# foundation-model-stack/fms-fsdp

Measured on AMD Instinct MI355X. Metric: tokens/sec (aggregate), higher is better.
Workload: dtype bf16; 1 GPU; model=llama2_7b, global_batch=2, seq_len=4096, parallelism=hsdp1

## Files before the change

fms_fsdp_amd/models/llama.py:

```python

import math
import os
from dataclasses import dataclass


import torch
import torch.nn as nn

from fms_fsdp_amd import ops


@dataclass
class LlamaConfig:
    src_vocab_size: int = 32000
    emb_dim: int = 4096
    nheads: int = 32
    kvheads: int = 0
    nlayers: int = 32
    hidden_grow_factor: float = 8 / 3
    multiple_of: int = 256
    max_expected_seq_len: int = 4096
    rope_theta: float = 10000.0
    norm_eps: float = 1e-6

# ... 47 lines not shown
        return freqs.cos(), freqs.sin()

    def get(self, seqlen, device):
        if seqlen > self.cos.shape[0]:
            cos, sin = self._build(seqlen)
            self.cos, self.sin = cos.to(device), sin.to(device)
        return self.cos[:seqlen], self.sin[:seqlen]

    def reset_parameters(self):
        cos, sin = self._build(self.max_seq_len)
        with torch.no_grad():
            self.cos.copy_(cos)
            self.sin.copy_(sin)


class Attention(nn.Module):
    def __init__(self, cfg: LlamaConfig):
        super().__init__()
        self.nheads = cfg.nheads
        self.kvheads = cfg.kvheads
        self.head_dim = cfg.head_dim
        qkv_out = (cfg.nheads + 2 * cfg.kvheads) * cfg.head_dim
        self.qkv = nn.Linear(cfg.emb_dim, qkv_out, bias=False)
        self.proj = nn.Linear(cfg.emb_dim, cfg.emb_dim, bias=False)
        self.qkv.weight._direct_wgrad = True
        self.proj.weight._direct_wgrad = True

    def _project_out(self, o2, residual, b, s):
        if getattr(self, "_disable_fused_residual", False):
            out = self.proj(o2.reshape(b * s, -1)).view(b, s, -1)
            return out if residual is None else out + residual
        return ops.linear_flat(o2.view(b, s, -1), self.proj.weight, residual)

    def forward(self, x, cos, sin, cache=None, residual=None, doc_mask=None):
        b, s, _ = x.shape
        if getattr(self, "_disable_fused_residual", False):
            qkv = self.qkv(x)
        else:
            qkv = ops.linear_flat(x, self.qkv.weight)
        if (cache is None and qkv.is_cuda and s % 128 == 0
                and self.head_dim in (64, 128)
                and qkv.dtype == torch.bfloat16
                and os.environ.get("FMS_AMD_ALLOW_TORCH_SDPA") != "1"
                and os.environ.get("FMS_AMD_DISABLE_FUSED_QKV") != "1"):
            o = ops.qkv_rope_attention(qkv, cos, sin, self.nheads,
                                       self.kvheads, self.head_dim,
                                       doc_mask=doc_mask)
            return self._project_out(o.reshape(b, s, -1), residual, b, s)
        q, k, v = qkv.split(
            [self.nheads * self.head_dim,
             self.kvheads * self.head_dim,
             self.kvheads * self.head_dim], dim=-1)
        q = q.view(b, s, self.nheads, self.head_dim)
        k = k.view(b, s, self.kvheads, self.head_dim)
        v = v.view(b, s, self.kvheads, self.head_dim)
        q, k = ops.rope_apply(q, k, cos, sin)
        if cache is not None:
            import torch.nn.functional as F
            if cache.get("k") is not None:
                k = torch.cat([cache["k"], k], dim=1)
                v = torch.cat([cache["v"], v], dim=1)
            cache["k"], cache["v"] = k, v
            o = F.scaled_dot_product_attention(
                q.transpose(1, 2), k.transpose(1, 2), v.transpose(1, 2),
                is_causal=(s == k.shape[1]),
                enable_gqa=(self.kvheads != self.nheads)).transpose(1, 2)
        else:
            o = ops.attention_causal(q, k, v, doc_mask=doc_mask)
        return self._project_out(o.reshape(b, s, -1), residual, b, s)

    def reset_parameters(self):
        for lin in (self.qkv, self.proj):
            nn.init.trunc_normal_(lin.weight, mean=0.0, std=0.02)


class SwiGLU(nn.Module):
    def __init__(self, cfg: LlamaConfig):
        super().__init__()
        self.hidden_dim = cfg.hidden_dim
        self.wg1 = nn.Linear(cfg.emb_dim, 2 * cfg.hidden_dim, bias=False)
        self.w2 = nn.Linear(cfg.hidden_dim, cfg.emb_dim, bias=False)
        self.wg1.weight._direct_wgrad = True
        self.w2.weight._direct_wgrad = True

    def forward(self, x, residual=None):
        if getattr(self, "_disable_fused_residual", False):
            gu = self.wg1(x)
            h = ops.swiglu(gu)
            out = self.w2(h)
            return out if residual is None else out + residual.view_as(out)
        gu = ops.linear_flat(x, self.wg1.weight)
        h = ops.swiglu(gu)
        return ops.linear_flat(h, self.w2.weight, residual)

    def reset_parameters(self):
        for lin in (self.wg1, self.w2):
            nn.init.trunc_normal_(lin.weight, mean=0.0, std=0.02)


class LlamaBlock(nn.Module):

    def __init__(self, cfg: LlamaConfig):
        super().__init__()
        self.attn_norm = RMSNorm(cfg.emb_dim, cfg.norm_eps)
        self.attn = Attention(cfg)
        self.mlp_norm = RMSNorm(cfg.emb_dim, cfg.norm_eps)
        self.mlp = SwiGLU(cfg)
        self.attn_norm.weight._direct_wgrad = True
        self.mlp_norm.weight._direct_wgrad = True

    def forward(self, x, cos, sin, cache=None, doc_mask=None):
        if cache is None and getattr(self, "_ac_enabled", False) \
                and torch.is_grad_enabled():
            return torch.utils.checkpoint.checkpoint(
                self._forward_impl, x, cos, sin, None, doc_mask,
                use_reentrant=False)
        return self._forward_impl(x, cos, sin, cache, doc_mask)

    def _forward_impl(self, x, cos, sin, cache=None, doc_mask=None):
        n, x_res = ops.rmsnorm_residual(x, self.attn_norm.weight,
                                        self.attn_norm.eps)
        h = self.attn(n, cos, sin, cache, residual=x_res, doc_mask=doc_mask)
        n, h_res = ops.rmsnorm_residual(h, self.mlp_norm.weight,
                                        self.mlp_norm.eps)
        return self.mlp(n, residual=h_res)

    def reset_parameters(self):
        for m in (self.attn_norm, self.attn, self.mlp_norm, self.mlp):
            m.reset_parameters()


class Llama(nn.Module):
    def __init__(self, cfg: LlamaConfig):
        super().__init__()
        self.config = cfg
        self.embedding = nn.Embedding(cfg.src_vocab_size, cfg.emb_dim)
        self.rot_emb = RotaryEmbedding(cfg.head_dim, cfg.max_expected_seq_len, cfg.rope_theta)
        self.layers = nn.ModuleList([LlamaBlock(cfg) for _ in range(cfg.nlayers)])
        self.norm = RMSNorm(cfg.emb_dim, cfg.norm_eps)
        self.norm.weight._direct_wgrad = True
        self.lm_head = nn.Linear(cfg.emb_dim, cfg.src_vocab_size, bias=False)
        self.doc_mask_token = None

    def forward(self, tokens, labels=None, include_embeds=False,
                doc_mask=None):
        b, s = tokens.shape
        if doc_mask is None and self.doc_mask_token is not None:
            doc_mask = ops.doc_mask_from_tokens(tokens, self.doc_mask_token)
        x = self.embedding(tokens)
        cos, sin = self.rot_emb.get(s, x.device)
        for layer in self.layers:
            x = layer(x, cos, sin, doc_mask=doc_mask)
        x = self.norm(x)
        if labels is not None:
            loss = ops.linear_cross_entropy(x, self.lm_head.weight, labels)
            return (loss, x) if include_embeds else loss
        logits = self.lm_head(x)
        return (logits, x) if include_embeds else logits

    @torch.no_grad()
    def generate(self, input_ids, max_new_tokens, temperature=1.0,
                 do_sample=True, include_embeds=False):
        b, s0 = input_ids.shape
        caches = [{} for _ in self.layers]
        tokens = input_ids
        embeds = []
# ... 38 lines not shown
```

fms_fsdp_amd/ops/__init__.py:

```python

import os
from typing import NamedTuple

import torch

from . import reference


_C = None
_C_err = None
try:
    from fms_fsdp_amd import _C
except ImportError as e:
    _C_err = e


def _require_ext(op):
    if _C is None:
        raise RuntimeError(
            f"fms_fsdp_amd._C HIP extension is required for {op} on GPU but "
            f"could not be imported ({_C_err}). Build it with "
            f"`python setup.py build_ext --inplace` (PYTORCH_ROCM_ARCH=gfx950)."
        )
    return _C
# ... 114 lines not shown
        weight = _WgradSinkFn.apply(weight)
    return reference.rmsnorm(x, weight, eps)


def rmsnorm_residual(x, weight, eps=1e-6):
    out = _rmsnorm_dispatch(_RMSNormResidualFn, x, weight, eps)
    if out is not None:
        return out
    if _direct_wgrad_on(weight):
        weight = _WgradSinkFn.apply(weight)
    return reference.rmsnorm(x, weight, eps), x


class _AddRMSNormFn(torch.autograd.Function):

    @staticmethod
    def forward(ctx, x, res, weight, eps):
        ext = _require_ext("add_rmsnorm")
        x2d = x.contiguous().view(-1, x.shape[-1])
        r2d = res.contiguous().view_as(x2d)
        y, s, rinv = ext.add_rmsnorm_fwd(x2d, r2d, weight, eps)
        ctx.save_for_backward(s, weight, rinv)
        ctx.shape = x.shape
        return y.view(x.shape), s.view(x.shape)

    @staticmethod
    def backward(ctx, dy, ds):
        s, weight, rinv = ctx.saved_tensors
        dx, dw = _C.rmsnorm_bwd(dy.contiguous().view_as(s), s, weight, rinv,
                                ds.contiguous().view_as(s))
        dx = dx.view(ctx.shape)
        return dx, dx, dw.to(weight.dtype), None


def add_rmsnorm(x, res, weight, eps=1e-6):
    if x.is_cuda and x.dtype != torch.float32:
        if x.dtype == torch.float16:
            y, s = _AddRMSNormFn.apply(x.bfloat16(), res.bfloat16(),
                                       weight.bfloat16(), eps)
            return y.half(), s.half()
        return _AddRMSNormFn.apply(x, res, weight, eps)
    s = (x.float() + res.float()).to(x.dtype)
    return reference.rmsnorm(s, weight, eps), s


def _row_view_ok(t):
    return (t.dim() == 4 and t.stride(3) == 1 and t.stride(2) == t.shape[3]
            and t.stride(1) >= t.shape[2] * t.shape[3]
            and t.stride(0) == t.shape[1] * t.stride(1))


def _as_row_view(t):
    return t if _row_view_ok(t) else t.contiguous()


class _RoPEFn(torch.autograd.Function):
    @staticmethod
    def forward(ctx, q, k, cos, sin):
        ext = _require_ext("rope")
        cos = cos.float().contiguous()
        sin = sin.float().contiguous()
        qo, ko = ext.rope_fwd(_as_row_view(q), _as_row_view(k), cos, sin,
                              False)
        ctx.save_for_backward(cos, sin)
        return qo, ko

    @staticmethod
    def backward(ctx, dq, dk):
        cos, sin = ctx.saved_tensors
        dqo, dko = _C.rope_fwd(_as_row_view(dq), _as_row_view(dk), cos, sin,
                               True)
        return dqo, dko, None, None


def rope_apply(q, k, cos, sin):
    if q.is_cuda and q.dtype != torch.float32:
        if q.dtype == torch.float16:
            qo, ko = _RoPEFn.apply(q.bfloat16(), k.bfloat16(), cos, sin)
            return qo.half(), ko.half()
        return _RoPEFn.apply(q, k, cos, sin)
    return reference.rope_apply(q, k, cos, sin)


class _DirectWgradLinearFn(torch.autograd.Function):
    @staticmethod
    def forward(ctx, x, weight, residual):
        ctx.save_for_backward(x, weight)
        ctx.gview = weight._flat_grad_view
        ctx.wobj = weight
        ctx.cb = getattr(weight, "_wgrad_done", None)
        ctx.res_shape = residual.shape if residual is not None else None
        x2 = x.reshape(-1, x.shape[-1])
        if residual is not None:
            y = torch.addmm(residual.reshape(x2.shape[0], -1), x2,
                            weight.t())
        else:
            y = x2 @ weight.t()
        return y.view(*x.shape[:-1], weight.shape[0])

    @staticmethod
    def backward(ctx, dy):
        x, w = ctx.saved_tensors
        dy2 = dy.reshape(-1, dy.shape[-1])
        x2 = x.reshape(-1, x.shape[-1])
        dx = (dy2 @ w).view(x.shape)
        if getattr(ctx.wobj, "_wgrad_fresh", False):
            torch.addmm(ctx.gview, dy2.t(), x2, beta=0, out=ctx.gview)
            ctx.wobj._wgrad_fresh = False
        else:
            ctx.gview.addmm_(dy2.t(), x2)
        if ctx.cb is not None:
            ctx.cb()
        dres = dy.reshape(ctx.res_shape) if ctx.res_shape is not None else None
        return dx, None, dres


def linear_flat(x, weight, residual=None):
    if (getattr(weight, "_flat_grad_view", None) is not None
            and weight.requires_grad and torch.is_grad_enabled()):
        return _DirectWgradLinearFn.apply(x, weight, residual)
    x2 = x.reshape(-1, x.shape[-1])
    if residual is not None:
        y = torch.addmm(residual.reshape(x2.shape[0], -1), x2, weight.t())
    else:
        y = x2 @ weight.t()
    return y.view(*x.shape[:-1], weight.shape[0])


class DocMask(NamedTuple):
    start: torch.Tensor
    end: torch.Tensor


def doc_mask_from_starts(doc_start):
    b, s = doc_start.shape
    start = doc_start.long()
    pos = torch.arange(s, device=start.device).expand(b, s)
    opens = torch.where(start == pos, pos, torch.full_like(pos, s))
    nxt = torch.cat([opens[:, 1:], torch.full_like(pos[:, :1], s)], dim=1)
    end = torch.cummin(nxt.flip(1), dim=1).values.flip(1)
    return DocMask(start.int().contiguous(), end.int().contiguous())


def doc_mask_from_tokens(tokens, eos_token):
    b, s = tokens.shape
    pos = torch.arange(s, device=tokens.device).expand(b, s)
    after = torch.where(tokens == eos_token, pos + 1, torch.zeros_like(pos))
    prev = torch.cat([torch.zeros_like(after[:, :1]), after[:, :-1]], dim=1)
    return doc_mask_from_starts(torch.cummax(prev, dim=1).values)


def _pad_doc_mask(doc_mask, s_pad):
    b, s = doc_mask.start.shape
    if s == s_pad:
        return doc_mask.start.contiguous(), doc_mask.end.contiguous()
    start = doc_mask.start.new_full((b, s_pad), s)
    end = doc_mask.end.new_full((b, s_pad), s_pad)
    start[:, :s] = doc_mask.start
    end[:, :s] = doc_mask.end
    return start, end


class _FlashAttnFn(torch.autograd.Function):

    @staticmethod
    def _pad(t, s_pad):
        b, s, h, d = t.shape
        if s == s_pad:
            return t.contiguous()
        out = torch.zeros(b, s_pad, h, d, dtype=t.dtype, device=t.device)
        out[:, :s] = t
        return out

    @staticmethod
    def forward(ctx, q, k, v, doc_start=None, doc_end=None):
        ext = _require_ext("attention")
        s = q.shape[1]
        s_pad = (s + 127) // 128 * 128
        qp = _FlashAttnFn._pad(q, s_pad)
        kp = _FlashAttnFn._pad(k, s_pad)
        vp = _FlashAttnFn._pad(v, s_pad)
        if doc_start is None:
            o, lse = ext.attn_fwd(qp, kp, vp)
            ctx.save_for_backward(qp, kp, vp, o, lse)
        else:
            o, lse = ext.attn_fwd_doc(qp, kp, vp, doc_start)
            ctx.save_for_backward(qp, kp, vp, o, lse, doc_start, doc_end)
        ctx.s = s
# ... 353 lines not shown
```

fms_fsdp_amd/ops/hip/bindings.cpp:

```cpp
#include <torch/extension.h>
#include <c10/hip/HIPStream.h>
#include <hip/hip_runtime_api.h>

#include <string>
#include <tuple>
#include <vector>

#include "attn_ws.h"

using torch::Tensor;

extern "C" {
void launch_rmsnorm_fwd(const void*, const void*, void*, float*, int, int,
                        float, hipStream_t);
void launch_rmsnorm_bwd(const void*, const void*, const void*, const float*,
                        const void*, void*, float*, int, int, hipStream_t);
void launch_add_rmsnorm_fwd(const void*, const void*, const void*, void*,
                            void*, float*, int, int, float, hipStream_t);
int rmsnorm_bwd_grid(int);
int rmsnorm_bwd_nparts(int, int);
void launch_rmsnorm_bwd_fused(const void*, const void*, const void*,
                              const float*, const void*, void*, float*, int,
                              float*, void*, int, int, int, hipStream_t);
void launch_rmsnorm_dw_store(const float*, void*, int, int, hipStream_t);
void launch_rope(const void*, void*, const float*, const float*, int, int,
                 int, int, int, long long, long long, hipStream_t);
void launch_swiglu_fwd(const void*, void*, long long, int, hipStream_t);
void launch_swiglu_bwd(const void*, const void*, void*, long long, int,
                       hipStream_t);
void launch_ce_fwd_bwd(void*, const long long*, float*, const float*,
                       long long, int, int, hipStream_t);
void launch_adamw(float*, const void*, int, float*, float*, void*, int,
                  long long, float, float, float, float, float, float, float,
                  const float*, hipStream_t);
void launch_sqnorm(const void*, int, float*, long long, hipStream_t);
void launch_attn_fwd(const void*, const void*, const void*, void*, float*,
                     int, int, int, int, int, float, long long, hipStream_t);
void launch_attn_bwd(const void*, const void*, const void*, const void*,
                     const void*, const float*, void*, void*, void*, float*,
                     void*, int, int, int, int, int, float, int,
                     long long, long long, hipStream_t);
void launch_attn_fwd_doc(const void*, const void*, const void*, void*, float*,
                         const int*, int, int, int, int, int, float,
                         long long, hipStream_t);
void launch_attn_bwd_doc(const void*, const void*, const void*, const void*,
                         const void*, const float*, void*, void*, void*,
                         float*, const int*, const int*, int, int, int, int,
                         int, float, int, long long, long long, hipStream_t);
void launch_attn_bwd_delta(const void*, const void*, float*, int, int, int,
                           int, hipStream_t);
int attn_sched_mode(int);
int attn_dkv_mode(int);
long long attn_bwd_ws_limit(long long);
void launch_cconv_fwd(const void*, const void*, const float*, void*, int,
                      int, int, int, hipStream_t);
void launch_cconv_bwd(const void*, const void*, const void*, const float*,
                      void*, void*, float*, float*, int, int, int, int,
                      hipStream_t);
int launch_gemm_nt(const void*, const void*, void*, int, int, int,
                   hipStream_t);
void launch_segsum_exp_fwd(const float*, void*, long long, int, hipStream_t);
void launch_segsum_exp_bwd(const void*, const float*, float*, long long, int,
                           hipStream_t);
void launch_ssd_prep_fwd(const void*, const float*, const float*, float*,
                         float*, long long, int, int, long long, hipStream_t);
void launch_ssd_prep_bwd(const float*, const float*, const void*,
                         const float*, const float*, void*, float*, float*,
                         long long, int, int, long long, long long,
                         hipStream_t);
void launch_ssd_xdt_fwd(const void*, const float*, const float*, void*, void*,
                        long long, int, int, int, long long, hipStream_t);
void launch_ssd_xdt_bwd(const void*, const void*, const void*, const float*,
                        const float*, void*, float*, float*, long long, int,
                        int, int, long long, long long, hipStream_t);
void launch_ssd_sl_fwd(const float*, const void*, void*, long long, int, int,
                       int, hipStream_t);
void launch_ssd_sl_bwd(const void*, const void*, const float*, void*, float*,
                       long long, int, int, int, hipStream_t);
void launch_ssd_ygate_fwd(const void*, const void*, const float*, const void*,
                          const float*, const void*, void*, long long, int,
                          int, int, int, long long, long long, hipStream_t);
void launch_ssd_ygate_bwd(const void*, const void*, const void*, const float*,
                          const void*, const float*, const void*, void*,
                          void*, float*, void*, float*, void*, long long, int,
                          int, int, int, long long, long long, long long,
                          long long, hipStream_t);
}

static hipStream_t cur_stream() {
  return c10::hip::getCurrentHIPStream().stream();
}

#define CHECK_BF16_CONTIG(t)                                        \
  TORCH_CHECK(t.scalar_type() == torch::kBFloat16, #t " must be bf16"); \
  TORCH_CHECK(t.is_contiguous(), #t " must be contiguous");

std::tuple<Tensor, Tensor> rmsnorm_fwd(Tensor x, Tensor w, double eps) {
  CHECK_BF16_CONTIG(x);
  CHECK_BF16_CONTIG(w);
  const int rows = x.size(0), H = x.size(1);
  TORCH_CHECK(H % 8 == 0, "H must be divisible by 8");
  auto y = torch::empty_like(x);
  auto rinv = torch::empty({rows}, x.options().dtype(torch::kFloat32));
  launch_rmsnorm_fwd(x.data_ptr(), w.data_ptr(), y.data_ptr(),
                     rinv.data_ptr<float>(), rows, H, (float)eps,
                     cur_stream());
  return {y, rinv};
}

static void check_rmsnorm_bwd_args(const Tensor& dy, const Tensor& x,
                                   const Tensor& w, const Tensor& rinv,
                                   const c10::optional<Tensor>& dextra) {
  CHECK_BF16_CONTIG(dy);
  CHECK_BF16_CONTIG(x);
  CHECK_BF16_CONTIG(w);
  TORCH_CHECK(x.dim() == 2 && dy.sizes() == x.sizes(),
              "dy and x must be (rows, H)");
  const int rows = x.size(0), H = x.size(1);
  TORCH_CHECK(H % 8 == 0, "H must be divisible by 8");
  TORCH_CHECK(w.numel() == H, "w must have H elements");
  TORCH_CHECK(rinv.scalar_type() == torch::kFloat32 && rinv.is_contiguous() &&
                  rinv.numel() == rows,
              "rinv must be fp32 with one element per row");
  if (dextra.has_value()) {
    TORCH_CHECK(dextra->scalar_type() == torch::kBFloat16 &&
                    dextra->is_contiguous() && dextra->sizes() == x.sizes(),
                "dextra must have x's shape and dtype");
  }
}

std::tuple<Tensor, Tensor> rmsnorm_bwd(Tensor dy, Tensor x, Tensor w,
                                       Tensor rinv,
                                       c10::optional<Tensor> dextra) {
  check_rmsnorm_bwd_args(dy, x, w, rinv, dextra);
  const int rows = x.size(0), H = x.size(1);
  const void* de = dextra.has_value() ? dextra->data_ptr() : nullptr;
  auto f32 = x.options().dtype(torch::kFloat32);
  auto dx = torch::empty_like(x);
  const int nparts = rmsnorm_bwd_nparts(rows, H);
  if (nparts == 0) {
    auto dw = torch::zeros({H}, f32);
    launch_rmsnorm_bwd(dy.data_ptr(), x.data_ptr(), w.data_ptr(),
                       rinv.data_ptr<float>(), de, dx.data_ptr(),
// ... 341 lines not shown
  } else {
    dv = out_bf16 ? torch::empty({b, s, kvh, d}, opts)
                  : torch::zeros({b, s, kvh, d}, opts);
  }
  auto delta = torch::empty({b, h, s}, q.options().dtype(torch::kFloat32));
  const float scale = 1.f / sqrtf((float)d);
  launch_attn_bwd_doc(do_.data_ptr(), q.data_ptr(), k.data_ptr(),
                      v.data_ptr(), o.data_ptr(), lse.data_ptr<float>(),
                      dq.data_ptr(), dk.data_ptr(), dv.data_ptr(),
                      delta.data_ptr<float>(), doc_start.data_ptr<int>(),
                      doc_end.data_ptr<int>(), b, s, h, kvh, d, scale,
                      out_bf16 ? 1 : 0, vs, dvs, cur_stream());
  if (out_bf16) return {dq, dk, dv};
  return {dq, dk.to(torch::kBFloat16), dv.to(torch::kBFloat16)};
}

Tensor cconv_fwd(Tensor x, Tensor w, Tensor bias) {
  CHECK_BF16_CONTIG(x);
  CHECK_BF16_CONTIG(w);
  const int b = x.size(0), l = x.size(1), c = x.size(2);
  const int W = w.size(1);
  TORCH_CHECK(c % 8 == 0 && W >= 2 && W <= 4);
  TORCH_CHECK(bias.scalar_type() == torch::kFloat32);
  auto y = torch::empty_like(x);
  launch_cconv_fwd(x.data_ptr(), w.data_ptr(), bias.data_ptr<float>(),
                   y.data_ptr(), b * l, l, c, W, cur_stream());
  return y;
}

std::tuple<Tensor, Tensor, Tensor> cconv_bwd(Tensor dy, Tensor x, Tensor w,
                                             Tensor bias) {
  CHECK_BF16_CONTIG(dy);
  CHECK_BF16_CONTIG(x);
  const int b = x.size(0), l = x.size(1), c = x.size(2);
  const int W = w.size(1);
  TORCH_CHECK(c % 8 == 0 && W >= 2 && W <= 4);
  auto g = torch::empty_like(x);
  auto dx = torch::empty_like(x);
  auto dw = torch::zeros({c, W}, x.options().dtype(torch::kFloat32));
  auto db = torch::zeros({c}, x.options().dtype(torch::kFloat32));
  launch_cconv_bwd(dy.data_ptr(), x.data_ptr(), w.data_ptr(),
                   bias.data_ptr<float>(), g.data_ptr(), dx.data_ptr(),
                   dw.data_ptr<float>(), db.data_ptr<float>(), b * l, l, c, W,
                   cur_stream());
  return {dx, dw, db};
}

Tensor segsum_exp_fwd(Tensor cs) {
  TORCH_CHECK(cs.scalar_type() == torch::kFloat32 && cs.is_contiguous());
  const long long N = cs.numel() / cs.size(-1);
  const int Q = cs.size(-1);
  TORCH_CHECK(Q % 8 == 0);
  std::vector<int64_t> shape(cs.sizes().begin(), cs.sizes().end());
  shape.push_back(Q);
  auto out = torch::empty(shape, cs.options().dtype(torch::kBFloat16));
  launch_segsum_exp_fwd(cs.data_ptr<float>(), out.data_ptr(), N, Q,
                        cur_stream());
  return out;
}

Tensor segsum_exp_bwd(Tensor g, Tensor cs) {
  CHECK_BF16_CONTIG(g);
  const long long N = cs.numel() / cs.size(-1);
  const int Q = cs.size(-1);
  auto dcs = torch::empty_like(cs);
  launch_segsum_exp_bwd(g.data_ptr(), cs.data_ptr<float>(),
                        dcs.data_ptr<float>(), N, Q, cur_stream());
  return dcs;
}


Tensor gemm_nt(Tensor A, Tensor B) {
  CHECK_BF16_CONTIG(A);
  CHECK_BF16_CONTIG(B);
  const int M = A.size(0), K = A.size(1), N = B.size(1);
  TORCH_CHECK(B.size(0) == K);
  auto C = torch::empty({M, N}, A.options());
  const int rc = launch_gemm_nt(A.data_ptr(), B.data_ptr(), C.data_ptr(), M,
                                N, K, cur_stream());
  TORCH_CHECK(rc == 0, "gemm_nt: shape not supported (M%256/N%256/K%64)");
  return C;
}

static long long slice_stride(const Tensor& t, const char* nm) {
  TORCH_CHECK(t.scalar_type() == torch::kBFloat16, nm, " must be bf16");
  TORCH_CHECK(t.dim() == 2 && t.stride(1) == 1, nm, " must be 2-D row-major");
  return t.stride(0);
}

static void check_nq(const Tensor& t, long long N, long long Q,
                     const char* nm) {
  TORCH_CHECK(t.scalar_type() == torch::kFloat32, nm, " must be fp32");
  TORCH_CHECK(t.is_contiguous(), nm, " must be contiguous");
  TORCH_CHECK(t.dim() == 2 && t.size(0) == N && t.size(1) == Q, nm,
              " must have shape (rows/Q*H, Q)");
}

static void check_bf16_numel(const Tensor& t, long long numel,
                             const char* nm) {
  TORCH_CHECK(t.scalar_type() == torch::kBFloat16, nm, " must be bf16");
  TORCH_CHECK(t.is_contiguous(), nm, " must be contiguous");
  TORCH_CHECK(t.numel() == numel, nm, " has the wrong element count");
}

static void check_head_vec(const Tensor& t, long long H, const char* nm) {
  TORCH_CHECK(t.scalar_type() == torch::kFloat32 && t.is_contiguous() &&
                  t.numel() == H,
              nm, " must be contiguous fp32 with H elements");
}

static long long check_xslice(const Tensor& t, int64_t H, int64_t P,
                              int64_t Q, const char* nm) {
  const long long st = slice_stride(t, nm);
  TORCH_CHECK(H > 0 && P > 0 && P % 8 == 0, "P must be divisible by 8");
  TORCH_CHECK(Q > 0 && Q % 8 == 0, "Q must be divisible by 8");
  TORCH_CHECK(t.size(1) == H * P, nm, " must have H*P columns");
  TORCH_CHECK(t.size(0) % Q == 0, nm, " rows must be a multiple of Q");
  return st;
}

static void check_prep_q(long long rows, int64_t Q) {
  TORCH_CHECK(Q > 0 && Q <= 256 && Q % 64 == 0 && rows % Q == 0,
              "Q must be 64, 128, 192 or 256 and divide the row count");
}

std::tuple<Tensor, Tensor> ssd_prep_fwd(Tensor dt, Tensor bias, Tensor alog,
                                        int64_t Q) {
  const long long sdt = slice_stride(dt, "dt");
  const long long rows = dt.size(0);
  const int H = dt.size(1);
  check_prep_q(rows, Q);
  check_head_vec(bias, H, "bias");
  check_head_vec(alog, H, "alog");
  const long long N = rows / Q * H;
  auto opt = dt.options().dtype(torch::kFloat32);
  auto dtf = torch::empty({N, Q}, opt);
  auto dacs = torch::empty({N, Q}, opt);
  launch_ssd_prep_fwd(dt.data_ptr(), bias.data_ptr<float>(),
                      alog.data_ptr<float>(), dtf.data_ptr<float>(),
                      dacs.data_ptr<float>(), N, H, (int)Q, sdt,
                      cur_stream());
  return {dtf, dacs};
}

std::tuple<Tensor, Tensor, Tensor> ssd_prep_bwd(Tensor ddtf, Tensor ddacs,
                                                Tensor dt, Tensor bias,
                                                Tensor alog, int64_t Q) {
  const long long sdt = slice_stride(dt, "dt");
  const long long rows = dt.size(0);
  const int H = dt.size(1);
  check_prep_q(rows, Q);
  check_head_vec(bias, H, "bias");
  check_head_vec(alog, H, "alog");
  const long long N = rows / Q * H;
  check_nq(ddtf, N, Q, "ddtf");
  check_nq(ddacs, N, Q, "ddacs");
  auto ddt = torch::empty({rows, (long long)H},
                          dt.options().dtype(torch::kBFloat16));
  auto dbias = torch::zeros({H}, dt.options().dtype(torch::kFloat32));
  auto dalog = torch::zeros({H}, dt.options().dtype(torch::kFloat32));
  launch_ssd_prep_bwd(ddtf.data_ptr<float>(), ddacs.data_ptr<float>(),
                      dt.data_ptr(), bias.data_ptr<float>(),
                      alog.data_ptr<float>(), ddt.data_ptr(),
                      dbias.data_ptr<float>(), dalog.data_ptr<float>(), N, H,
                      (int)Q, sdt, H, cur_stream());
  return {ddt, dbias, dalog};
// ... 69 lines not shown
  const int Q = check_sl(dacs, scores, H, G);
  const long long N = dacs.size(0);
  check_bf16_numel(g, N * Q * Q, "g");
  auto dsh = torch::empty({N, (long long)Q, (long long)Q}, g.options());
  auto dcs = torch::zeros_like(dacs);
  launch_ssd_sl_bwd(g.data_ptr(), scores.data_ptr(), dacs.data_ptr<float>(),
                    dsh.data_ptr(), dcs.data_ptr<float>(), N, (int)H, (int)G,
                    Q, cur_stream());
  return {dsh, dcs};
}

static void check_ygate(const Tensor& ydiag, const Tensor& yoff,
                        const Tensor& dacs, const Tensor& x, const Tensor& Dp,
                        const Tensor& z, int64_t H, int64_t G, int64_t Q) {
  TORCH_CHECK(G > 0 && H % G == 0, "H must be a multiple of G");
  TORCH_CHECK(z.size(0) == x.size(0), "x and z must have the same rows");
  check_bf16_numel(ydiag, x.numel(), "ydiag");
  check_bf16_numel(yoff, x.numel(), "yoff");
  check_nq(dacs, x.size(0) / Q * H, Q, "dacs");
  check_head_vec(Dp, H, "D");
}

Tensor ssd_ygate_fwd(Tensor ydiag, Tensor yoff, Tensor dacs, Tensor x,
                     Tensor Dp, Tensor z, int64_t H, int64_t G, int64_t P,
                     int64_t Q) {
  const long long sx = check_xslice(x, H, P, Q, "x");
  const long long sz = check_xslice(z, H, P, Q, "z");
  const long long rows = x.size(0);
  check_ygate(ydiag, yoff, dacs, x, Dp, z, H, G, Q);
  auto out = torch::empty({rows, H * P}, x.options().dtype(torch::kBFloat16));
  launch_ssd_ygate_fwd(ydiag.data_ptr(), yoff.data_ptr(),
                       dacs.data_ptr<float>(), x.data_ptr(),
                       Dp.data_ptr<float>(), z.data_ptr(), out.data_ptr(),
                       rows * H * P / 8, (int)H, (int)G, (int)Q, (int)P, sx,
                       sz, cur_stream());
  return out;
}

std::vector<Tensor> ssd_ygate_bwd(Tensor dout, Tensor ydiag, Tensor yoff,
                                  Tensor dacs, Tensor x, Tensor Dp, Tensor z,
                                  int64_t H, int64_t G, int64_t P,
                                  int64_t Q) {
  const long long sx = check_xslice(x, H, P, Q, "x");
  const long long sz = check_xslice(z, H, P, Q, "z");
  const long long rows = x.size(0);
  check_ygate(ydiag, yoff, dacs, x, Dp, z, H, G, Q);
  check_bf16_numel(dout, rows * H * P, "dout");
  auto o = x.options().dtype(torch::kBFloat16);
  auto dydiag = torch::empty({rows, H * P}, o);
  auto dyoff = torch::empty({rows, H * P}, o);
  auto ddacs = torch::empty_like(dacs);
  auto dx = torch::empty({rows, H * P}, o);
  auto dD_rows = torch::empty({rows, H}, x.options().dtype(torch::kFloat32));
  auto dz = torch::empty({rows, H * P}, o);
  launch_ssd_ygate_bwd(dout.data_ptr(), ydiag.data_ptr(), yoff.data_ptr(),
                       dacs.data_ptr<float>(), x.data_ptr(),
                       Dp.data_ptr<float>(), z.data_ptr(), dydiag.data_ptr(),
                       dyoff.data_ptr(), ddacs.data_ptr<float>(),
                       dx.data_ptr(), dD_rows.data_ptr<float>(),
                       dz.data_ptr(), rows * H, (int)H, (int)G, (int)Q,
                       (int)P, sx, sz, H * P, H * P, cur_stream());
  return {dydiag, dyoff, ddacs, dx, dD_rows, dz};
}

PYBIND11_MODULE(TORCH_EXTENSION_NAME, mod) {
  mod.def("segsum_exp_fwd", &segsum_exp_fwd);
  mod.def("segsum_exp_bwd", &segsum_exp_bwd);
  mod.def("cconv_fwd", &cconv_fwd);
  mod.def("cconv_bwd", &cconv_bwd);
  mod.def("rmsnorm_fwd", &rmsnorm_fwd);
  mod.def("rmsnorm_bwd", &rmsnorm_bwd);
  mod.def("rmsnorm_bwd_into", &rmsnorm_bwd_into);
  mod.def("rmsnorm_bwd_grid", &rmsnorm_bwd_grid_py,
          pybind11::arg("grid") = pybind11::none());
  mod.def("add_rmsnorm_fwd", &add_rmsnorm_fwd);
  mod.def("rope_fwd", &rope_fwd);
  mod.def("rope_into", &rope_into);
  mod.def("swiglu_fwd", &swiglu_fwd);
  mod.def("swiglu_bwd", &swiglu_bwd);
  mod.def("ce_fwd_bwd", &ce_fwd_bwd);
  mod.def("adamw", &adamw);
  mod.def("sq_norm_accum", &sq_norm_accum);
  mod.def("gemm_nt", &gemm_nt);
  mod.def("ssd_prep_fwd", &ssd_prep_fwd);
  mod.def("ssd_prep_bwd", &ssd_prep_bwd);
  mod.def("ssd_xdt_fwd", &ssd_xdt_fwd);
  mod.def("ssd_xdt_bwd", &ssd_xdt_bwd);
  mod.def("ssd_sl_fwd", &ssd_sl_fwd);
  mod.def("ssd_sl_bwd", &ssd_sl_bwd);
  mod.def("ssd_ygate_fwd", &ssd_ygate_fwd);
  mod.def("ssd_ygate_bwd", &ssd_ygate_bwd);
  mod.def("attn_fwd", &attn_fwd);
  mod.def("attn_bwd", &attn_bwd);
  mod.def("attn_bwd_delta", &attn_bwd_delta);
  mod.def("attn_fwd_doc", &attn_fwd_doc);
  mod.def("attn_bwd_doc", &attn_bwd_doc);
  mod.def("attn_sched_mode", &attn_sched_mode_py,
          pybind11::arg("mode") = pybind11::none());
  mod.def("attn_dkv_mode", &attn_dkv_mode_py,
          pybind11::arg("mode") = pybind11::none());
  mod.def("attn_bwd_ws_limit", &attn_bwd_ws_limit_py,
          pybind11::arg("bytes") = pybind11::none());
}
```

fms_fsdp_amd/parallel/fsdp.py:

```python

import os
from contextlib import nullcontext
from typing import List, Optional, Type

import torch
import torch.distributed as dist
import torch.nn as nn

from fms_fsdp_amd import ops

_ALIGN = 128


def _pad_to(n, k):
    return (n + k - 1) // k * k


class FlatUnit:

    def __init__(self, name: str, module: nn.Module, params: List[nn.Parameter],
                 shard_group, replicate_group, device, param_dtype,
                 reshard_after_forward: bool, param_names=None,
                 reduce_dtype=None):
        self.name = name
# ... 174 lines not shown
        return sum(p.numel() for p in self.params)


class ShardedModel(nn.Module):

    def __init__(self, model: nn.Module, block_class: Type[nn.Module],
                 sharding_strategy: str = "fsdp",
                 device=None,
                 param_dtype=torch.bfloat16,
                 reduce_dtype=torch.bfloat16,
                 reshard_after_forward: bool = False,
                 prefetch_lookahead: int = 1,
                 intra_node_size: Optional[int] = None):
        super().__init__()
        self.model = model
        self.prefetch_lookahead = max(prefetch_lookahead, 0)
        self.reduce_dtype = reduce_dtype
        self._step_trained = False

        world = dist.get_world_size() if dist.is_initialized() else 1
        rank = dist.get_rank() if dist.is_initialized() else 0
        if device is None:
            device = torch.device("cuda", torch.cuda.current_device()) \
                if torch.cuda.is_available() else torch.device("cpu")
        self.device = device
        self.is_cuda = device.type == "cuda"

        shard_group = replicate_group = None
        if world > 1:
            if sharding_strategy == "fsdp":
                shard_group = dist.group.WORLD
            elif sharding_strategy == "hsdp":
                intra = intra_node_size or int(os.environ.get("LOCAL_WORLD_SIZE", 0)) \
                    or min(world, torch.cuda.device_count() or world)
                if world % intra != 0:
                    intra = world
                mesh_shard, mesh_rep = _build_hsdp_groups(world, rank, intra)
                shard_group, replicate_group = mesh_shard, mesh_rep
                if dist.get_world_size(shard_group) == 1:
                    shard_group = None
                if replicate_group is not None and \
                        dist.get_world_size(replicate_group) == 1:
                    replicate_group = None
            elif sharding_strategy == "ddp":
                shard_group = None
                replicate_group = dist.group.WORLD
            else:
                raise ValueError(f"unknown sharding strategy {sharding_strategy}")
        self.shard_group = shard_group
        self.replicate_group = replicate_group

        blocks = [(n, m) for n, m in model.named_modules() if isinstance(m, block_class)]
        name_of = {id(p): n for n, p in model.named_parameters()}
        block_param_ids = set()
        self.units: List[FlatUnit] = []
        for n, m in blocks:
            params = [p for p in m.parameters() if p.requires_grad]
            block_param_ids.update(id(p) for p in params)
            self.units.append(FlatUnit(n, m, params, shard_group, replicate_group,
                                       device, param_dtype, reshard_after_forward,
                                       param_names=[name_of[id(p)] for p in params],
                                       reduce_dtype=reduce_dtype))
        root_params = [p for p in model.parameters()
                       if p.requires_grad and id(p) not in block_param_ids]
        self.root_unit = None
        if root_params:
            self.root_unit = FlatUnit(
                "_root", model, root_params, shard_group, replicate_group,
                device, param_dtype, False,
                param_names=[name_of[id(p)] for p in root_params],
                reduce_dtype=reduce_dtype)
        self.all_units = ([self.root_unit] if self.root_unit else []) \
            + self.units
        self._unit_of_module = {id(u.module): u for u in self.units}

        if any(p.is_meta for p in model.parameters()):
            self._materialize_from_meta()
        else:
            for b in model.buffers():
                b.data = b.data.to(device)
            for u in self.all_units:
                u.materialize(src_rank_broadcast=True)
        self._pool_unit_storage()

        self.comm_stream = torch.cuda.Stream() if self.is_cuda else None
        self.rs_stream = torch.cuda.Stream() if self.is_cuda else None

        self._install_hooks()

    def _pool_unit_storage(self):
        units = self.all_units
        if not units:
            return
        dev = self.device
        S = units[0].S

        def pool(attr, dtype, sizes):
            total = sum(sizes)
            buf = torch.empty(total, dtype=dtype, device=dev)
            off = 0
            views = []
            for u, n in zip(units, sizes):
                v = buf[off:off + n]
                v.copy_(getattr(u, attr))
                views.append(v)
                off += n
            return buf, views

        sizes = [u.shard_size for u in units]
        for attr, dt in (("master_shard", torch.float32),
                         ("exp_avg", torch.float32),
                         ("exp_avg_sq", torch.float32)):
            buf, views = pool(attr, dt, sizes)
            setattr(self, "_pool_" + attr, buf)
            for u, v in zip(units, views):
                setattr(u, attr, v)
        if S > 1:
            pdt = units[0].param_dtype
            rdt = units[0].reduce_dtype
            self._pool_param_shard, views = pool("param_shard", pdt, sizes)
            for u, v in zip(units, views):
                u.param_shard = v
            self._pool_grad_shard, views = pool("grad_shard", rdt, sizes)
            for u, v in zip(units, views):
                u.grad_shard = v
        else:
            totals = [u.total for u in units]
            pdt = units[0].param_dtype
            self._pool_param_shard, views = pool("flat_param", pdt, totals)
            for u, v in zip(units, views):
                u.flat_param = v
                u.param_shard = v
                u._point_params_into_flat()
            self._pool_grad_shard, gviews = pool("flat_grad", pdt, totals)
            rdt = units[0].reduce_dtype
            sep_reduce = rdt != pdt
            for u, v in zip(units, gviews):
                u.flat_grad = v
                if not sep_reduce:
                    u.grad_shard = v
                u._set_grad_views()
            if sep_reduce:
                self._pool_reduce_shard, views = pool("grad_shard", rdt, totals)
                for u, v in zip(units, views):
                    u.grad_shard = v

    def _pooled_grad_norm_src(self):
        units = self.all_units
        if units and units[0].S == 1 and \
                units[0].grad_shard is not units[0].flat_grad:
            return self._pool_reduce_shard
        return self._pool_grad_shard

    def _materialize_from_meta(self):
        model, dev = self.model, self.device
        slot_of = {}
        for m in model.modules():
            for n, p in m.named_parameters(recurse=False):
                slot_of[id(p)] = (m, n)
        for m in model.modules():
            if any(b.is_meta for b in m.buffers(recurse=False)) and \
                    not any(True for _ in m.parameters(recurse=False)):
                m.to_empty(device=dev, recurse=False)
                if hasattr(m, "reset_parameters"):
                    m.reset_parameters()
        for u in self.all_units:
            slots = [slot_of[id(p)] for p in u.params]
            owners = []
            for m, _ in slots:
                if m not in owners:
                    owners.append(m)
            for m in owners:
                m.to_empty(device=dev, recurse=False)
            if u is self.root_unit and hasattr(model, "reset_root_parameters"):
                model.reset_root_parameters()
            elif u is not self.root_unit and hasattr(u.module, "reset_parameters"):
                u.module.reset_parameters()
            else:
                for m in owners:
                    if hasattr(m, "reset_parameters"):
                        m.reset_parameters()
            for (m, n), old in zip(slots, u.params):
                if getattr(old, "_direct_wgrad", False):
                    m._parameters[n]._direct_wgrad = True
            u.params = [m._parameters[n] for m, n in slots]
            u.materialize(src_rank_broadcast=True)
        for b in model.buffers():
            if b.is_meta:
                raise RuntimeError("meta buffer left unmaterialized — give "
                                   "its module a reset_parameters()")
            if b.device != dev:
                b.data = b.data.to(dev)


    def _install_hooks(self):
        for i, u in enumerate(self.units):
            u.module.register_forward_pre_hook(self._make_fwd_pre(i))
            u.module.register_forward_hook(self._make_fwd_post(i))
            u.module.register_full_backward_pre_hook(self._make_bwd_pre(i))
        for u in self.all_units:
            for p in u.params:
                if getattr(p, "_direct_wgrad", False):
                    p._wgrad_done = self._make_wgrad_cb(u)
                else:
                    p.register_post_accumulate_grad_hook(
                        self._make_grad_hook(u))

    def _make_fwd_pre(self, idx):
        def hook(module, args):
            u = self.units[idx]
            u.gather(self.comm_stream)
            u.wait_gather()
            for j in range(idx + 1, min(idx + 1 + self.prefetch_lookahead,
                                        len(self.units))):
                self.units[j].gather(self.comm_stream)
        return hook

    def _make_fwd_post(self, idx):
        def hook(module, args, out):
            u = self.units[idx]
            if u.reshard_after_forward and torch.is_grad_enabled():
                u._free_flat_param()
            return None
        return hook

    def _make_bwd_pre(self, idx):
        def hook(module, grad_output):
            u = self.units[idx]
            u.prepare_grads()
            if not u._gathered:
                u.gather(self.comm_stream)
            u.wait_gather()
            for j in range(idx - 1, max(idx - 1 - self.prefetch_lookahead, -1), -1):
                if self.units[j].reshard_after_forward:
                    self.units[j].gather(self.comm_stream)
            if u._grad_countdown == 0:
                u._grad_countdown = len(u.params)
            return None
        return hook

    def _dec_grad(self, u: FlatUnit):
        if u._grad_countdown == 0:
            u._grad_countdown = len(u.params)
        u._grad_countdown -= 1
        if u._grad_countdown == 0:
            u.reduce_grads(self.rs_stream)
            if u.reshard_after_forward:
                u._free_flat_param()
                u.free_flat_grad(self.rs_stream)

    def _make_grad_hook(self, u: FlatUnit):
        def hook(param):
            self._dec_grad(u)
        return hook

    def _make_wgrad_cb(self, u: FlatUnit):
        def cb():
            self._dec_grad(u)
        return cb

    def forward(self, *args, **kwargs):
        if self.root_unit is not None:
            self.root_unit.gather(self.comm_stream)
            self.root_unit.wait_gather()
        for j in range(min(self.prefetch_lookahead, len(self.units))):
            self.units[j].gather(self.comm_stream)
        return self.model(*args, **kwargs)


    def clip_grad_norm_(self, max_norm):
        for u in self.all_units:
            u.wait_grads()
        local = ops.sq_norm([self._pooled_grad_norm_src()])
        if self.shard_group is not None:
            dist.all_reduce(local, group=self.shard_group)
        total_norm = local.sqrt()
        self._clip_coef = torch.clamp(max_norm / (total_norm + 1e-6), max=1.0)
        return total_norm

    def zero_grad(self, set_to_none=False):
        self._clip_coef = None
        for u in self.all_units:
            if u.flat_grad.untyped_storage().size() == 0:
                continue
            direct = [p for p in u.params
                      if getattr(p, "_direct_wgrad", False)]
            if not direct:
                u.flat_grad.zero_()
            else:
                for p, off in zip(u.params, u.offsets):
                    if getattr(p, "_direct_wgrad", False):
                        p._wgrad_fresh = True
                    else:
                        u.flat_grad[off:off + p.numel()].zero_()
            if u.grad_shard is not u.flat_grad:
                u.grad_shard.zero_()
            if not u._grads_ready_views:
                u._set_grad_views()

    def param_count(self):
        return sum(u.sharded_numel_unpadded() for u in self.all_units)


class ShardedAdamW:

    def __init__(self, sharded_model: ShardedModel, lr=3e-4, betas=(0.9, 0.95),
                 eps=1e-8, weight_decay=0.1):
        self.m = sharded_model
        self.lr = lr
        self.betas = betas
        self.eps = eps
        self.weight_decay = weight_decay
        self.step_count = 0
        self.param_groups = [{"lr": lr, "initial_lr": lr}]
        self.defaults = {"lr": lr}

    def step(self):
        self.step_count += 1
        lr = self.param_groups[0]["lr"]
        b1, b2 = self.betas
        gscale = getattr(self.m, "_clip_coef", None)
        m = self.m
        for u in m.all_units:
            u.wait_grads()
        pdt = m._pool_param_shard.dtype
        lowp = pdt in (torch.bfloat16, torch.float16)
        published = ops.fused_adamw(
            m._pool_master_shard, m._pooled_grad_norm_src(),
            m._pool_exp_avg, m._pool_exp_avg_sq,
            self.step_count, lr, b1, b2, self.eps, self.weight_decay,
            grad_scale=gscale,
            p_bf16_out=m._pool_param_shard if lowp else None)
        if not published or not lowp:
            with torch.no_grad():
                m._pool_param_shard.copy_(m._pool_master_shard)
        for u in m.all_units:
            u.mark_stale()

    def zero_grad(self, set_to_none=False):
        self.m.zero_grad()

    def state_dict(self):
        return {
            "step": self.step_count,
            "lr": self.param_groups[0]["lr"],
            "units": {u.name: {"exp_avg": u.exp_avg, "exp_avg_sq": u.exp_avg_sq,
                               "master": u.master_shard}
                      for u in self.m.all_units},
        }

    def load_state_dict(self, sd):
        self.step_count = sd["step"]
        self.param_groups[0]["lr"] = sd["lr"]
        for u in self.m.all_units:
            usd = sd["units"][u.name]
            u.exp_avg.copy_(usd["exp_avg"])
            u.exp_avg_sq.copy_(usd["exp_avg_sq"])
            u.master_shard.copy_(usd["master"])
            u.publish_master_to_shard()
            u.mark_stale()


class DynamicGradScaler:

    def __init__(self, enabled=True, init_scale=2.0 ** 16, growth_factor=2.0,
                 backoff_factor=0.5, growth_interval=1000):
        self.enabled = enabled
        self.scale = float(init_scale) if enabled else 1.0
        self.growth_factor = growth_factor
        self.backoff_factor = backoff_factor
        self.growth_interval = growth_interval
        self._good_steps = 0

    def scale_loss(self, loss):
        return loss * self.scale if self.enabled else loss

    def clip_and_step(self, model, optimizer, max_norm):
        if not self.enabled:
            gnorm = model.clip_grad_norm_(max_norm)
            optimizer.step()
            return gnorm, True
        gnorm_scaled = model.clip_grad_norm_(max_norm * self.scale)
        true_norm = gnorm_scaled / self.scale
        if not bool(torch.isfinite(gnorm_scaled)):
            self.scale = max(self.scale * self.backoff_factor, 1.0)
            self._good_steps = 0
            return true_norm, False
        model._clip_coef = model._clip_coef / self.scale
        optimizer.step()
        self._good_steps += 1
        if self._good_steps % self.growth_interval == 0:
            self.scale *= self.growth_factor
        return true_norm, True

    def state_dict(self):
        return {"scale": self.scale, "good_steps": self._good_steps,
                "enabled": self.enabled}

    def load_state_dict(self, sd):
        self.scale = sd["scale"]
        self._good_steps = sd["good_steps"]
        self.enabled = sd["enabled"]


def _build_hsdp_groups(world, rank, intra):
    n_nodes = world // intra
    shard_group = replicate_group = None
    for node in range(n_nodes):
        ranks = list(range(node * intra, (node + 1) * intra))
        g = dist.new_group(ranks)
        if rank in ranks:
            shard_group = g
    for local in range(intra):
        ranks = list(range(local, world, intra))
        g = dist.new_group(ranks)
        if rank in ranks:
            replicate_group = g
    return shard_group, replicate_group
```

setup.py:

```python

import os
import subprocess

from setuptools import setup
from torch.utils.cpp_extension import BuildExtension, CppExtension

ARCH = os.environ.get("PYTORCH_ROCM_ARCH", "gfx950")
ROCM = os.environ.get("ROCM_HOME", "/opt/rocm")
REPO = os.path.dirname(os.path.abspath(__file__))
HIP_DIR = os.path.join(REPO, "fms_fsdp_amd", "ops", "hip")
BUILD_DIR = os.path.join(REPO, "build", "hip_objs")

HIP_SOURCES = ["rmsnorm.hip", "rope.hip", "swiglu.hip", "cross_entropy.hip",
               "adamw.hip", "attention.hip", "causal_conv1d.hip", "ssd.hip",
               "gemm_nt.hip"]
HIP_HEADERS = ["common.h", "attn_sched.h", "attn_ws.h"]


def compile_hip_objects():
    os.makedirs(BUILD_DIR, exist_ok=True)
    objs = []
    for src in HIP_SOURCES:
        src_path = os.path.join(HIP_DIR, src)
        obj_path = os.path.join(BUILD_DIR, src.replace(".hip", ".o"))
        deps = [src_path] + [os.path.join(HIP_DIR, h) for h in HIP_HEADERS]
        if (not os.path.exists(obj_path)
                or any(os.path.getmtime(obj_path) < os.path.getmtime(d)
                       for d in deps)):
            cmd = [os.path.join(ROCM, "bin", "hipcc"),
                   f"--offload-arch={ARCH}", "-O3", "-std=c++17", "-fPIC",
                   "-c", src_path, "-o", obj_path]
            print(" ".join(cmd))
            subprocess.check_call(cmd)
        objs.append(obj_path)
    return objs


class HipBuildExt(BuildExtension):
    def build_extensions(self):
        objs = compile_hip_objects()
        for ext in self.extensions:
            ext.extra_objects = objs + list(ext.extra_objects or [])
        super().build_extensions()


setup(
    name="fms_fsdp_amd",
    packages=["fms_fsdp_amd"],
    ext_modules=[
        CppExtension(
            name="fms_fsdp_amd._C",
            sources=[os.path.join("fms_fsdp_amd", "ops", "hip", "bindings.cpp")],
            extra_compile_args=["-O3", "-std=c++17",
                                "-D__HIP_PLATFORM_AMD__=1", "-DUSE_ROCM=1"],
            include_dirs=[os.path.join(ROCM, "include")],
            library_dirs=[os.path.join(ROCM, "lib")],
            libraries=["amdhip64", "c10_hip", "torch_hip"],
        )
    ],
    cmdclass={"build_ext": HipBuildExt},
)
```

Measured before the change: 22880 tokens/s.

## Pre-transpose MLP weights into scratch buffer for backward dgrad GEMMs

Adds a batched tiled bf16 transpose kernel and uses it to transpose each unit's SwiGLU weights into a shared scratch buffer when the unit is gathered in backward. The dgrad matmul then multiplies dy by a transposed view of that pre-transposed copy, so the GEMM sees an NT layout that may map to faster hipBLASLt kernels than the NN form. In exchange it adds an extra pass over the weights per unit, a scratch buffer sized to the largest unit, and owner tracking that must be reset on forward and optimizer steps.

New measurement: 23100 tokens/s (median of 6 runs). About the same (+1.0%).

```diff
diff --git a/fms_fsdp_amd/models/llama.py b/fms_fsdp_amd/models/llama.py
--- a/fms_fsdp_amd/models/llama.py
+++ b/fms_fsdp_amd/models/llama.py
@@ -153,6 +153,8 @@
         self.w2 = nn.Linear(cfg.hidden_dim, cfg.emb_dim, bias=False)
         self.wg1.weight._direct_wgrad = True
         self.w2.weight._direct_wgrad = True
+        self.wg1.weight._dgrad_transposed = True
+        self.w2.weight._dgrad_transposed = True
 
     def forward(self, x, residual=None):
         if getattr(self, "_disable_fused_residual", False):
diff --git a/fms_fsdp_amd/ops/__init__.py b/fms_fsdp_amd/ops/__init__.py
--- a/fms_fsdp_amd/ops/__init__.py
+++ b/fms_fsdp_amd/ops/__init__.py
@@ -220,6 +220,28 @@
     return reference.rope_apply(q, k, cos, sin)
 
 
+
+DGRAD_MODE = os.environ.get("FMS_AMD_DGRAD", "transposed")
+if DGRAD_MODE not in ("direct", "transposed"):
+    raise ValueError(f"FMS_AMD_DGRAD: expected 'direct' or 'transposed', "
+                     f"got '{DGRAD_MODE}'")
+
+
+class DgradScratch:
+
+    def __init__(self):
+        self.buf = None
+        self.owner = None
+
+
+def _dgrad_transposed(weight):
+    ref = getattr(weight, "_dgrad_t", None)
+    if ref is None or DGRAD_MODE != "transposed":
+        return None
+    scratch, unit, wt = ref
+    return wt if scratch.owner is unit else None
+
+
 class _DirectWgradLinearFn(torch.autograd.Function):
     @staticmethod
     def forward(ctx, x, weight, residual):
@@ -241,7 +263,11 @@
         x, w = ctx.saved_tensors
         dy2 = dy.reshape(-1, dy.shape[-1])
         x2 = x.reshape(-1, x.shape[-1])
-        dx = (dy2 @ w).view(x.shape)
+        wt = _dgrad_transposed(ctx.wobj)
+        if wt is not None:
+            dx = torch.mm(dy2, wt.t()).view(x.shape)
+        else:
+            dx = (dy2 @ w).view(x.shape)
         if getattr(ctx.wobj, "_wgrad_fresh", False):
             torch.addmm(ctx.gview, dy2.t(), x2, beta=0, out=ctx.gview)
             ctx.wobj._wgrad_fresh = False
diff --git a/fms_fsdp_amd/ops/hip/bindings.cpp b/fms_fsdp_amd/ops/hip/bindings.cpp
--- a/fms_fsdp_amd/ops/hip/bindings.cpp
+++ b/fms_fsdp_amd/ops/hip/bindings.cpp
@@ -2,6 +2,8 @@
 #include <c10/hip/HIPStream.h>
 #include <hip/hip_runtime_api.h>
 
+#include <algorithm>
+#include <cstdint>
 #include <string>
 #include <tuple>
 #include <vector>
@@ -59,6 +61,9 @@
                       hipStream_t);
 int launch_gemm_nt(const void*, const void*, void*, int, int, int,
                    hipStream_t);
+int launch_transpose_batched(const void* const*, void* const*,
+                             const long long*, const long long*, int,
+                             hipStream_t);
 void launch_segsum_exp_fwd(const float*, void*, long long, int, hipStream_t);
 void launch_segsum_exp_bwd(const void*, const float*, float*, long long, int,
                            hipStream_t);
@@ -566,6 +571,45 @@
   return C;
 }
 
+void transpose_into(std::vector<Tensor> srcs, std::vector<Tensor> dsts) {
+  TORCH_CHECK(srcs.size() == dsts.size(),
+              "transpose_into: srcs and dsts differ in length");
+  const size_t n = srcs.size();
+  if (n == 0) return;
+  for (size_t i = 0; i < n; ++i) {
+    const Tensor& s = srcs[i];
+    const Tensor& d = dsts[i];
+    TORCH_CHECK(s.is_cuda() && d.is_cuda() && s.device() == srcs[0].device() &&
+                    d.device() == s.device(),
+                "transpose_into: all tensors must be on one GPU");
+    TORCH_CHECK(s.scalar_type() == torch::kBFloat16 &&
+                    d.scalar_type() == torch::kBFloat16,
+                "transpose_into: src and dst must be bf16");
+    TORCH_CHECK(s.dim() == 2 && d.dim() == 2 && s.size(0) >= 1 &&
+                    s.size(1) >= 1 && s.size(0) <= INT32_MAX &&
+                    s.size(1) <= INT32_MAX,
+                "transpose_into: src must be 2-D with R, C >= 1");
+    TORCH_CHECK(d.size(0) == s.size(1) && d.size(1) == s.size(0),
+                "transpose_into: dst must have shape (C, R)");
+    TORCH_CHECK(s.is_contiguous() && d.is_contiguous(),
+                "transpose_into: src and dst must be contiguous");
+  }
+  for (size_t base = 0; base < n; base += 8) {
+    const int m = (int)std::min<size_t>(8, n - base);
+    const void* sp[8];
+    void* dp[8];
+    long long R[8], C[8];
+    for (int i = 0; i < m; ++i) {
+      sp[i] = srcs[base + i].data_ptr();
+      dp[i] = dsts[base + i].data_ptr();
+      R[i] = srcs[base + i].size(0);
+      C[i] = srcs[base + i].size(1);
+    }
+    const int rc = launch_transpose_batched(sp, dp, R, C, m, cur_stream());
+    TORCH_CHECK(rc == 0, "transpose_into: too many tiles for one launch");
+  }
+}
+
 static long long slice_stride(const Tensor& t, const char* nm) {
   TORCH_CHECK(t.scalar_type() == torch::kBFloat16, nm, " must be bf16");
   TORCH_CHECK(t.dim() == 2 && t.stride(1) == 1, nm, " must be 2-D row-major");
@@ -801,6 +845,7 @@
   mod.def("adamw", &adamw);
   mod.def("sq_norm_accum", &sq_norm_accum);
   mod.def("gemm_nt", &gemm_nt);
+  mod.def("transpose_into", &transpose_into);
   mod.def("ssd_prep_fwd", &ssd_prep_fwd);
   mod.def("ssd_prep_bwd", &ssd_prep_bwd);
   mod.def("ssd_xdt_fwd", &ssd_xdt_fwd);
diff --git a/fms_fsdp_amd/ops/hip/transpose.hip b/fms_fsdp_amd/ops/hip/transpose.hip
--- /dev/null
+++ b/fms_fsdp_amd/ops/hip/transpose.hip
@@ -0,0 +1,111 @@
+#include "common.h"
+
+#define TP_TILE 64
+#define TP_MAX 8
+
+struct TransposeArgs {
+  const unsigned short* src[TP_MAX];
+  unsigned short* dst[TP_MAX];
+  int R[TP_MAX];
+  int C[TP_MAX];
+  int tiles_c[TP_MAX];
+  int start[TP_MAX];
+  int fast[TP_MAX];
+  int n;
+};
+
+__device__ __forceinline__ int tp_lds_index(int r, int c) {
+  return r * TP_TILE + ((((c >> 3) ^ (r >> 3)) & 7) << 3) + (c & 7);
+}
+
+__global__ __launch_bounds__(256) void transpose_batched_kernel(
+    const TransposeArgs a) {
+  __shared__ __attribute__((aligned(16))) unsigned short tile[TP_TILE * TP_TILE];
+
+  const int b = blockIdx.x;
+  const unsigned short* src = a.src[0];
+  unsigned short* dst = a.dst[0];
+  int R = a.R[0], C = a.C[0], tc_n = a.tiles_c[0], first = 0, fast = a.fast[0];
+#pragma unroll
+  for (int i = 1; i < TP_MAX; ++i) {
+    if (i < a.n && b >= a.start[i]) {
+      src = a.src[i];
+      dst = a.dst[i];
+      R = a.R[i];
+      C = a.C[i];
+      tc_n = a.tiles_c[i];
+      first = a.start[i];
+      fast = a.fast[i];
+    }
+  }
+  const int t = b - first;
+  const int r0 = (t / tc_n) * TP_TILE;
+  const int c0 = (t % tc_n) * TP_TILE;
+  const int tid = threadIdx.x;
+
+  if (fast) {
+#pragma unroll
+    for (int p = 0; p < 2; ++p) {
+      const int i = tid + p * 256;
+      const int r = i >> 3, v = i & 7;
+      const bf16x8 x = *reinterpret_cast<const bf16x8*>(
+          src + (size_t)(r0 + r) * C + c0 + v * 8);
+      *reinterpret_cast<bf16x8*>(
+          &tile[r * TP_TILE + ((v ^ (r >> 3)) & 7) * 8]) = x;
+    }
+    __syncthreads();
+#pragma unroll
+    for (int p = 0; p < 2; ++p) {
+      const int i = tid + p * 256;
+      const int c = i >> 3, g = i & 7;
+      bf16x8 y;
+#pragma unroll
+      for (int j = 0; j < 8; ++j)
+        y.v[j] = (short)tile[tp_lds_index(g * 8 + j, c)];
+      *reinterpret_cast<bf16x8*>(dst + (size_t)(c0 + c) * R + r0 + g * 8) = y;
+    }
+    return;
+  }
+
+  for (int i = tid; i < TP_TILE * TP_TILE; i += 256) {
+    const int r = i >> 6, c = i & 63;
+    if (r0 + r < R && c0 + c < C)
+      tile[tp_lds_index(r, c)] = src[(size_t)(r0 + r) * C + c0 + c];
+  }
+  __syncthreads();
+  for (int i = tid; i < TP_TILE * TP_TILE; i += 256) {
+    const int c = i >> 6, r = i & 63;
+    if (r0 + r < R && c0 + c < C)
+      dst[(size_t)(c0 + c) * R + r0 + r] = tile[tp_lds_index(r, c)];
+  }
+}
+
+extern "C" {
+
+int launch_transpose_batched(const void* const* src, void* const* dst,
+                             const long long* R, const long long* C, int n,
+                             hipStream_t stream) {
+  TransposeArgs a = {};
+  long long blocks = 0;
+  for (int i = 0; i < n; ++i) {
+    const long long tr = (R[i] + TP_TILE - 1) / TP_TILE;
+    const long long tc = (C[i] + TP_TILE - 1) / TP_TILE;
+    a.src[i] = (const unsigned short*)src[i];
+    a.dst[i] = (unsigned short*)dst[i];
+    a.R[i] = (int)R[i];
+    a.C[i] = (int)C[i];
+    a.tiles_c[i] = (int)tc;
+    a.start[i] = (int)blocks;
+    a.fast[i] = R[i] % TP_TILE == 0 && C[i] % TP_TILE == 0 &&
+                ((uintptr_t)src[i] & 15) == 0 && ((uintptr_t)dst[i] & 15) == 0;
+    blocks += tr * tc;
+    if (blocks > 0x7fffffffLL) return -1;
+  }
+  a.n = n;
+  if (blocks == 0) return 0;
+  transpose_batched_kernel<<<(unsigned)blocks, 256, 0, stream>>>(a);
+  HIP_CHECK_LAUNCH();
+  return 0;
+}
+
+}
diff --git a/fms_fsdp_amd/parallel/fsdp.py b/fms_fsdp_amd/parallel/fsdp.py
--- a/fms_fsdp_amd/parallel/fsdp.py
+++ b/fms_fsdp_amd/parallel/fsdp.py
@@ -280,6 +280,7 @@
             for u in self.all_units:
                 u.materialize(src_rank_broadcast=True)
         self._pool_unit_storage()
+        self._plan_dgrad_scratch()
 
         self.comm_stream = torch.cuda.Stream() if self.is_cuda else None
         self.rs_stream = torch.cuda.Stream() if self.is_cuda else None
@@ -343,6 +344,42 @@
                 for u, v in zip(units, views):
                     u.grad_shard = v
 
+    def _plan_dgrad_scratch(self):
+        self._dgrad = ops.DgradScratch()
+        self._dgrad_numel = 0
+        for u in self.units:
+            u._dgrad_routed = []
+        if not self.is_cuda:
+            return
+        for u in self.units:
+            if u.param_dtype != torch.bfloat16:
+                continue
+            off = 0
+            for p in u.params:
+                if getattr(p, "_direct_wgrad", False) and p.dim() == 2 \
+                        and getattr(p, "_dgrad_transposed", False):
+                    u._dgrad_routed.append((p, off))
+                    off += _pad_to(p.numel(), _ALIGN)
+            self._dgrad_numel = max(self._dgrad_numel, off)
+
+    def _transpose_unit_weights(self, u: FlatUnit):
+        d = self._dgrad
+        if not u._dgrad_routed or ops.DGRAD_MODE != "transposed":
+            return
+        d.owner = None
+        if d.buf is None:
+            d.buf = torch.empty(self._dgrad_numel, dtype=torch.bfloat16,
+                                device=self.device)
+        srcs, dsts = [], []
+        for p, off in u._dgrad_routed:
+            if getattr(p, "_dgrad_t", None) is None:
+                n, k = p.shape
+                p._dgrad_t = (d, u, d.buf[off:off + n * k].view(k, n))
+            srcs.append(p.data)
+            dsts.append(p._dgrad_t[2])
+        ops._require_ext("transpose_into").transpose_into(srcs, dsts)
+        d.owner = u
+
     def _pooled_grad_norm_src(self):
         units = self.all_units
         if units and units[0].S == 1 and \
@@ -381,6 +418,8 @@
             for (m, n), old in zip(slots, u.params):
                 if getattr(old, "_direct_wgrad", False):
                     m._parameters[n]._direct_wgrad = True
+                if getattr(old, "_dgrad_transposed", False):
+                    m._parameters[n]._dgrad_transposed = True
             u.params = [m._parameters[n] for m, n in slots]
             u.materialize(src_rank_broadcast=True)
         for b in model.buffers():
@@ -429,6 +468,7 @@
             if not u._gathered:
                 u.gather(self.comm_stream)
             u.wait_gather()
+            self._transpose_unit_weights(u)
             for j in range(idx - 1, max(idx - 1 - self.prefetch_lookahead, -1), -1):
                 if self.units[j].reshard_after_forward:
                     self.units[j].gather(self.comm_stream)
@@ -458,6 +498,7 @@
         return cb
 
     def forward(self, *args, **kwargs):
+        self._dgrad.owner = None
         if self.root_unit is not None:
             self.root_unit.gather(self.comm_stream)
             self.root_unit.wait_gather()
@@ -534,6 +575,7 @@
                 m._pool_param_shard.copy_(m._pool_master_shard)
         for u in m.all_units:
             u.mark_stale()
+        m._dgrad.owner = None
 
     def zero_grad(self, set_to_none=False):
         self.m.zero_grad()
@@ -557,6 +599,7 @@
             u.master_shard.copy_(usd["master"])
             u.publish_master_to_shard()
             u.mark_stale()
+        self.m._dgrad.owner = None
 
 
 class DynamicGradScaler:
diff --git a/setup.py b/setup.py
--- a/setup.py
+++ b/setup.py
@@ -13,7 +13,7 @@
 
 HIP_SOURCES = ["rmsnorm.hip", "rope.hip", "swiglu.hip", "cross_entropy.hip",
                "adamw.hip", "attention.hip", "causal_conv1d.hip", "ssd.hip",
-               "gemm_nt.hip"]
+               "gemm_nt.hip", "transpose.hip"]
 HIP_HEADERS = ["common.h", "attn_sched.h", "attn_ws.h"]
 
 
```
